# MisEty/RTG-SLAM

Hardware: AMD Instinct MI355X
Metric: hot_path_units_per_sec (higher is better)
Workload: dtype f32; 1 GPU; `value` counts UNITS, not SLAM frames (the SLAM frame rate by the reference's definition is `slam_frames_per_sec`, from the `slam_sequence` leg of --full).  One UNIT per step = 1 ICP track (3 levels x 5 GN iters, 1200x680, on a second HIP stream) + 1 map-optimisation iteration (raster fwd + masked L1 colour / gated depth loss + attach regulariser + raster bwd + fused Adam) over 1200000 random Gaus; gaussians=1200000, mode=single, parallelism=1 GPU

## Files before the change

### include/rtgs_icp.h

```cpp
#ifndef RTGS_ICP_H
#define RTGS_ICP_H

#include <stddef.h>
#include <stdint.h>

#ifdef __cplusplus
extern "C" {
#endif

#define RTGS_ICP_MAX_LEVELS 8


int rtgs_icp_build_pyramids(const float* depth, int32_t H, int32_t W, const float* K, int32_t levels,
                            float* const* vertex_out_host, float* const* normal_out_host,
                            void* scratch, void* stream);

int rtgs_icp_scratch_init(void* scratch, void* stream);
#define RTGS_ICP_PYR_SCRATCH_READY 1
#define RTGS_ICP_PYR_SECOND_SET 2
int rtgs_icp_build_pyramids_ex(const float* depth, int32_t H, int32_t W, const float* K, int32_t levels,
                               float* const* vertex_out_host, float* const* normal_out_host,
                               void* scratch, int32_t flags, void* stream);

int rtgs_icp_step(const float* vertex_src, const float* normal_src, const float* vertex_tgt,
                  const float* normal_tgt, int32_t H, int32_t W, const float* K, const float* pose,
                  float distance_threshold, float cos_normal_threshold,
                  float* JtJ_out, float* Jtr_out, float* nvalid_out, void* scratch, void* stream);

typedef struct rtgs_icp_level {
  int32_t H, W;
  float downscale;
  int32_t iters;
  const float* vertex_src;
  const float* normal_src;
  const float* vertex_tgt;
  const float* normal_tgt;
} rtgs_icp_level;

int rtgs_icp_track(const rtgs_icp_level* levels_host, int32_t n_levels, const float* K,
                   float distance_threshold, float cos_normal_threshold, float damping,
                   float* pose_inout, float* stats_out, void* scratch, int32_t flags, void* stream);
#define RTGS_ICP_FLAG_PERSISTENT 1
#define RTGS_ICP_FLAG_SCRATCH_READY 4
#define RTGS_ICP_FLAG_FROM_IDENTITY 8
#define RTGS_ICP_FLAG_F32_SOLVE 16
#define RTGS_ICP_FLAG_CLUSTER 2

int rtgs_icp_fill_model_depth(float* render_depth, const float* frame_depth, const float* render_normal,
                              const float* frame_normal, int32_t H, int32_t W, float dist_thr,
                              float normal_thr, void* stream);

size_t rtgs_icp_scratch_bytes(void);

#ifdef __cplusplus
}
#endif
#endif
```

### rtg_slam_amd/csrc/icp.hip

```cpp
#include "../../include/rtgs_icp.h"
#include "../../include/rtgs_debug.h"
#include <hip/hip_runtime.h>
#include <math.h>
#include <stdlib.h>

namespace rtgs_icp {

#ifndef RTGS_ICP_MAX_BLOCKS
#define RTGS_ICP_MAX_BLOCKS 256
#endif
constexpr int MAX_BLOCKS = RTGS_ICP_MAX_BLOCKS;
static_assert(MAX_BLOCKS <= RTGS_ICP_STAMP_WGS, "stamp slots hold RTGS_ICP_STAMP_WGS workgroups");
constexpr int NACC = 28;
constexpr int PSTRIDE = 32;

struct Scratch {
  uint32_t minmax[2 * RTGS_ICP_MAX_LEVELS];
  float partials[MAX_BLOCKS * PSTRIDE];
  uint32_t ticket;
  uint32_t pad[15];
  double sums[24 * 8 * PSTRIDE];
  unsigned long long dbg[96];
  uint32_t minmax_b[2 * RTGS_ICP_MAX_LEVELS];
};

#ifndef RTGS_ICP_WAVE_PRIO
#define RTGS_ICP_WAVE_PRIO 3
#endif
__device__ __forceinline__ void wave_priority_high() {
#if RTGS_ICP_WAVE_PRIO > 0
  __builtin_amdgcn_s_setprio(RTGS_ICP_WAVE_PRIO);
#endif
}

__device__ __forceinline__ uint32_t enc_f(float f) {
  const uint32_t u = __float_as_uint(f);
  return (u & 0x80000000u) ? ~u : (u | 0x80000000u);
}
__device__ __forceinline__ float dec_f(uint32_t e) {
  return __uint_as_float((e & 0x80000000u) ? (e & 0x7fffffffu) : ~e);
}

struct PyrDesc {
  int levels;
  int H, W;
  int Hl[RTGS_ICP_MAX_LEVELS], Wl[RTGS_ICP_MAX_LEVELS], shift[RTGS_ICP_MAX_LEVELS];
  int block_start[RTGS_ICP_MAX_LEVELS + 1];
  float* vertex[RTGS_ICP_MAX_LEVELS];
  float* normal[RTGS_ICP_MAX_LEVELS];
  uint32_t* mm;
  uint32_t* mm_rearm;
};

__global__ void __launch_bounds__(256) icp_vertex_kernel(PyrDesc d, const float* __restrict__ depth,
                                                         const float* __restrict__ K, Scratch* sc) {
  __shared__ uint32_t s_mm[2 * RTGS_ICP_MAX_LEVELS];
  if (threadIdx.x < 2 * RTGS_ICP_MAX_LEVELS) s_mm[threadIdx.x] = 0xffffffffu;
  __syncthreads();
  const int total = d.block_start[d.levels];
  for (int chunk = blockIdx.x; chunk < total; chunk += gridDim.x) {
    int l = 0;
    while (l + 1 < d.levels && chunk >= d.block_start[l + 1]) ++l;
    const int Hl = d.Hl[l], Wl = d.Wl[l], sh = d.shift[l];
    const int idx = (chunk - d.block_start[l]) * 256 + (int)threadIdx.x;
    float dmax = 0.f;
    const bool live = idx < Hl * Wl;
    if (live) {
      const int y = idx / Wl, x = idx % Wl;
      const int f = 1 << sh;
      dmax = -INFINITY;
      for (int a = 0; a < f; ++a)
        for (int b = 0; b < f; ++b) dmax = fmaxf(dmax, depth[(size_t)(y * f + a) * d.W + (x * f + b)]);
      const float ds = 1.f / (float)f;
      const float fx = K[0] * ds, fy = K[4] * ds, cx = K[2] * ds, cy = K[5] * ds;
      float* v = d.vertex[l] + (size_t)idx * 3;
      v[0] = (((float)x - cx) / fx) * dmax;
// ... 111 lines not shown
    if ((threadIdx.x & 63) == 0 && a != 0xffffffffu) { atomicMin(&s_mm[2 * l], a); atomicMin(&s_mm[2 * l + 1], bq); }
  }
  __syncthreads();
  if (threadIdx.x < 6 && s_mm[threadIdx.x] != 0xffffffffu) atomicMin(&d.mm[threadIdx.x], s_mm[threadIdx.x]);
  if (d.mm_rearm && blockIdx.x == 0 && threadIdx.x < 6) d.mm_rearm[threadIdx.x] = 0xffffffffu;
}

__global__ void __launch_bounds__(256) icp_normal_kernel(PyrDesc d, const Scratch* sc) {
  wave_priority_high();
  int l = 0;
  while (l + 1 < d.levels && (int)blockIdx.x >= d.block_start[l + 1]) ++l;
  const int Hl = d.Hl[l], Wl = d.Wl[l];
  const int idx = ((int)blockIdx.x - d.block_start[l]) * 256 + (int)threadIdx.x;
  if (idx >= Hl * Wl) return;
  const int y = idx / Wl, x = idx % Wl;
  const float* V = d.vertex[l];
  const int ym = max(y - 1, 0), yp = min(y + 1, Hl - 1), xm = max(x - 1, 0), xp = min(x + 1, Wl - 1);
  float gx[3], gy[3];
#pragma unroll
  for (int c = 0; c < 3; ++c) {
    const float a00 = V[((size_t)ym * Wl + xm) * 3 + c], a01 = V[((size_t)ym * Wl + x) * 3 + c], a02 = V[((size_t)ym * Wl + xp) * 3 + c];
    const float a10 = V[((size_t)y * Wl + xm) * 3 + c], a12 = V[((size_t)y * Wl + xp) * 3 + c];
    const float a20 = V[((size_t)yp * Wl + xm) * 3 + c], a21 = V[((size_t)yp * Wl + x) * 3 + c], a22 = V[((size_t)yp * Wl + xp) * 3 + c];
    gx[c] = -a00 + a02 - 2.f * a10 + 2.f * a12 - a20 + a22;
    gy[c] = -a00 - 2.f * a01 - a02 + a20 + 2.f * a21 + a22;
  }
  float nx = __fmaf_rn(gy[1], gx[2], -(gy[2] * gx[1]));
  float ny = __fmaf_rn(gy[2], gx[0], -(gy[0] * gx[2]));
  float nz = __fmaf_rn(gy[0], gx[1], -(gy[1] * gx[0]));
  const float mag = sqrtf(__fmaf_rn(nz, nz, __fmaf_rn(ny, ny, nx * nx))) + 1e-8f;
  nx /= mag; ny /= mag; nz /= mag;
  const float dep = V[(size_t)idx * 3 + 2];
  const float dmin = dec_f(d.mm[2 * l]), dmax = dec_f(~d.mm[2 * l + 1]);
  if (dep <= dmin || dep >= dmax) { nx = 0.f; ny = 0.f; nz = 0.f; }
  float* N = d.normal[l] + (size_t)idx * 3;
  N[0] = nx; N[1] = ny; N[2] = nz;
}

template <int CTRL, int ROW_MASK = 0xf>
__device__ __forceinline__ float dpp_add(float v) {
  const int moved = __builtin_amdgcn_update_dpp(0, __float_as_int(v), CTRL, ROW_MASK, 0xf, false);
  return v + __int_as_float(moved);
}
__device__ __forceinline__ float wave_sum63(float v) {
  v = dpp_add<0xB1>(v);
  v = dpp_add<0x4E>(v);
  v = dpp_add<0x141>(v);
  v = dpp_add<0x140>(v);
  v = dpp_add<0x142, 0xa>(v);
  v = dpp_add<0x143, 0xc>(v);
  return v;
}

template <int NCOL>
__device__ __forceinline__ void block_write_partials(float (&acc)[NCOL], float* __restrict__ partials) {
  __shared__ float s_part[4 * PSTRIDE];
  const int lane = threadIdx.x & 63, wave = threadIdx.x >> 6;
#pragma unroll
  for (int k = 0; k < NCOL; ++k) {
    const float r = wave_sum63(acc[k]);
    if (lane == 63) s_part[wave * PSTRIDE + k] = r;
  }
  __syncthreads();
  if (threadIdx.x < NCOL) {
    const int k = threadIdx.x;
    __hip_atomic_store(&partials[(size_t)blockIdx.x * PSTRIDE + k],
                       (s_part[k] + s_part[PSTRIDE + k]) + (s_part[2 * PSTRIDE + k] + s_part[3 * PSTRIDE + k]),
                       __ATOMIC_RELAXED, __HIP_MEMORY_SCOPE_AGENT);
  }
}

__device__ __forceinline__ void block_add_totals(float (&acc)[NACC], double* __restrict__ totals) {
  __shared__ float s_part2[4 * PSTRIDE];
  const int lane = threadIdx.x & 63, wave = threadIdx.x >> 6;
#pragma unroll
  for (int k = 0; k < NACC; ++k) {
    const float r = wave_sum63(acc[k]);
    if (lane == 63) s_part2[wave * PSTRIDE + k] = r;
  }
  __syncthreads();
  if (threadIdx.x < NACC) {
    const int k = threadIdx.x;
    const float v = (s_part2[k] + s_part2[PSTRIDE + k]) + (s_part2[2 * PSTRIDE + k] + s_part2[3 * PSTRIDE + k]);
    if (v != 0.f) unsafeAtomicAdd(&totals[k], (double)v);
  }
}

enum { MODE_SOLVE = 0, MODE_EQUATIONS = 1, MODE_P2P = 2 };

__device__ __forceinline__ float ld_sc1(const float* p) {
  return __hip_atomic_load(p, __ATOMIC_RELAXED, __HIP_MEMORY_SCOPE_AGENT);
}

struct FinalArgs {
  int mode;
  float damping, inv_pixels;
  float* pose;
  float* stats;
  float* JtJ_out;
  float* Jtr_out;
  float* nvalid_out;
  int first;
  int f32_solve;
};

__device__ __forceinline__ void sum_partials(const float* __restrict__ partials, int nblocks, double* s_sum, double* s_tot) {
  {
    const int q = threadIdx.x & 7, grp = threadIdx.x >> 3;
    double a0 = 0.0, a1 = 0.0, a2 = 0.0, a3 = 0.0;
    if (q < 7) {
      constexpr int MAXR = (MAX_BLOCKS + 31) / 32;
      float t[MAXR][4];
#pragma unroll
      for (int i = 0; i < MAXR; ++i) {
        const int r = grp + 32 * i;
        if (r < nblocks) {
          const float* row = partials + (size_t)r * PSTRIDE + 4 * q;
          t[i][0] = ld_sc1(row); t[i][1] = ld_sc1(row + 1); t[i][2] = ld_sc1(row + 2); t[i][3] = ld_sc1(row + 3);
        } else {
          t[i][0] = t[i][1] = t[i][2] = t[i][3] = 0.f;
        }
      }
#pragma unroll
      for (int i = 0; i < MAXR; ++i) { a0 += (double)t[i][0]; a1 += (double)t[i][1]; a2 += (double)t[i][2]; a3 += (double)t[i][3]; }
    }
    s_sum[grp * PSTRIDE + 4 * q] = a0; s_sum[grp * PSTRIDE + 4 * q + 1] = a1;
    s_sum[grp * PSTRIDE + 4 * q + 2] = a2; s_sum[grp * PSTRIDE + 4 * q + 3] = a3;
  }
  __syncthreads();
  if (threadIdx.x < NACC) {
    double t = 0.0;
#pragma unroll
    for (int g = 0; g < 32; ++g) t += s_sum[g * PSTRIDE + threadIdx.x];
    s_tot[threadIdx.x] = t;
  }
  __syncthreads();
}

__device__ __forceinline__ bool gn_update(const double (&S)[NACC], float damping, const float (&pin)[16], float* pose) {
  double Hm[6][6], bvec[6];
#pragma unroll
  for (int r = 0; r < 6; ++r)
#pragma unroll
    for (int c = r; c < 6; ++c) {
      const int idx = r * 6 - (r * (r - 1)) / 2 + (c - r);
      Hm[r][c] = S[idx]; Hm[c][r] = S[idx];
    }
#pragma unroll
  for (int r = 0; r < 6; ++r) bvec[r] = S[21 + r];
  double tr = 0.0;
#pragma unroll
  for (int r = 0; r < 6; ++r) tr += Hm[r][r];
#pragma unroll
  for (int r = 0; r < 6; ++r) Hm[r][r] += tr * (double)damping;
  double L[6][6], inv[6];
  bool spd = true;
#pragma unroll
  for (int r = 0; r < 6; ++r) {
#pragma unroll
    for (int c = 0; c <= r; ++c) {
      double s = Hm[r][c];
#pragma unroll
      for (int m = 0; m < c; ++m) s -= L[r][m] * L[c][m];
      if (r == c) {
        spd = spd && (s > 0.0);
        L[r][r] = sqrt(s > 0.0 ? s : 1.0);
        inv[r] = 1.0 / L[r][r];
      } else {
        L[r][c] = s * inv[c];
      }
    }
  }
  if (!spd) return false;
  double yv[6], xi[6];
#pragma unroll
  for (int r = 0; r < 6; ++r) {
    double s = -bvec[r];
// ... 164 lines not shown
        const int lo = r < c ? r : c, hi = r < c ? c : r;
        fa.JtJ_out[r * 6 + c] = (float)S[lo * 6 - (lo * (lo - 1)) / 2 + (hi - lo)];
      }
      fa.Jtr_out[r] = (float)S[21 + r];
    }
    fa.nvalid_out[0] = (float)S[27];
    return;
  }
  if (fa.first & 1) { fa.stats[1] = 0.f; fa.stats[2] = 0.f; fa.stats[3] = 0.f; }
  if (fa.first & 2) {
#pragma unroll
    for (int k = 0; k < 16; ++k) fa.pose[k] = (k % 5 == 0) ? 1.f : 0.f;
  }
  fa.stats[0] = (float)(S[27] * (double)fa.inv_pixels);
  if (!(fa.f32_solve ? gn_update_f32(S, fa.damping, pin, fa.pose) : gn_update(S, fa.damping, pin, fa.pose))) fa.stats[2] += 1.f;
}

template <bool STAMP>
__device__ __forceinline__ void final_stage(const float* __restrict__ partials, int nblocks, const FinalArgs& fa,
                                            unsigned long long (&cyc)[2]) {
  __shared__ double s_sum[32 * PSTRIDE];
  __shared__ double s_tot[PSTRIDE];
  unsigned long long t0 = 0;
  if constexpr (STAMP) t0 = __builtin_readcyclecounter();
  float pin[16];
#pragma unroll
  for (int k = 0; k < 16; ++k) pin[k] = (k % 5 == 0) ? 1.f : 0.f;
  if (threadIdx.x == 0 && fa.mode == MODE_SOLVE && !(fa.first & 2)) {
#pragma unroll
    for (int k = 0; k < 16; ++k) pin[k] = fa.pose[k];
  }
  sum_partials(partials, nblocks, s_sum, s_tot);
  if constexpr (STAMP) { const unsigned long long t = __builtin_readcyclecounter(); cyc[0] = t - t0; t0 = t; }
  if (threadIdx.x != 0) return;
  final_solve_from(s_tot, fa, pin);
  if constexpr (STAMP) {
    asm volatile("s_waitcnt vmcnt(0)" ::: "memory");
    cyc[1] = __builtin_readcyclecounter() - t0;
  }
}

__device__ __forceinline__ bool arrive_and_elect_last(uint32_t* ticket) {
  __shared__ uint32_t s_is_last;
  asm volatile("s_waitcnt vmcnt(0)" ::: "memory");
  __syncthreads();
  if (threadIdx.x == 0) {
    const uint32_t t = __hip_atomic_fetch_add(ticket, 1u, __ATOMIC_RELAXED, __HIP_MEMORY_SCOPE_AGENT);
    const uint32_t last = (t == gridDim.x - 1) ? 1u : 0u;
    if (last) __hip_atomic_store(ticket, 0u, __ATOMIC_RELAXED, __HIP_MEMORY_SCOPE_AGENT);
    s_is_last = last;
  }
  __syncthreads();
  return s_is_last != 0;
}

struct LevelGeom {
  float R00, R01, R02, t0, R10, R11, R12, t1, R20, R21, R22, t2;
  float fx, fy, cx, cy, Wm1, Hm1, hw, hh, dist_thr, cos_thr;
  int W;
};

struct Proj {
  float px, py, pz;
  int j;
};
struct Tgt {
  float q0, q1, q2, m0, m1, m2;
};

__device__ __forceinline__ Proj project(const LevelGeom& g, float v0, float v1, float v2) {
  Proj P;
  P.px = (g.R00 * v0 + g.R01 * v1 + g.R02 * v2) + g.t0;
  P.py = (g.R10 * v0 + g.R11 * v1 + g.R12 * v2) + g.t1;
  P.pz = (g.R20 * v0 + g.R21 * v1 + g.R22 * v2) + g.t2;
  P.j = -1;
  const float u = (P.px / P.pz) * g.fx + g.cx;
  const float v = (P.py / P.pz) * g.fy + g.cy;
  const bool inview = (u > 0.f) && (u < g.Wm1) && (v > 0.f) && (v < g.Hm1);
  if (inview && (v2 > 0.f)) {
    const float un = u / g.hw - 1.f, vn = v / g.hh - 1.f;
    float ix = ((un + 1.f) / 2.f) * g.Wm1, iy = ((vn + 1.f) / 2.f) * g.Hm1;
    ix = fminf(g.Wm1, fmaxf(ix, 0.f));
    iy = fminf(g.Hm1, fmaxf(iy, 0.f));
    P.j = ((int)nearbyintf(iy) * g.W + (int)nearbyintf(ix)) * 3;
  }
  return P;
}

__device__ __forceinline__ Tgt gather(const Proj& P, const float* __restrict__ vt, const float* __restrict__ nt) {
  const int j = P.j < 0 ? 0 : P.j;
  return Tgt{vt[j], vt[j + 1], vt[j + 2], nt[j], nt[j + 1], nt[j + 2]};
}

__device__ __forceinline__ void finish(const LevelGeom& g, const Proj& P, float n0, float n1, float n2, const Tgt& T,
                                       float (&acc)[NACC]) {
  if (P.j < 0 || !(T.q2 > 0.f)) return;
  const float rn0 = g.R00 * n0 + g.R01 * n1 + g.R02 * n2;
  const float rn1 = g.R10 * n0 + g.R11 * n1 + g.R12 * n2;
  const float rn2 = g.R20 * n0 + g.R21 * n1 + g.R22 * n2;
  if (!(rn0 * T.m0 + rn1 * T.m1 + rn2 * T.m2 > g.cos_thr)) return;
  const float d0 = P.px - T.q0, d1 = P.py - T.q1, d2 = P.pz - T.q2;
  if (sqrtf(d0 * d0 + d1 * d1 + d2 * d2) > g.dist_thr) return;
  const float r = T.m0 * d0 + T.m1 * d1 + T.m2 * d2;
  float J[6];
  J[0] = P.py * T.m2 - P.pz * T.m1;
  J[1] = P.pz * T.m0 - P.px * T.m2;
// ... 66 lines not shown
  if (idx < n) {
    const float* v = vs + (size_t)idx * 3;
    const float* m = ns + (size_t)idx * 3;
    const float n0 = m[0], n1 = m[1], n2 = m[2];
    const Proj P = project(g, v[0], v[1], v[2]);
    finish(g, P, n0, n1, n2, gather(P, vt, nt), acc);
  }
}

template <bool STAMP>
__device__ __forceinline__ void icp_reduce_body(
    const float* __restrict__ vs, const float* __restrict__ ns, const float* __restrict__ vt,
    const float* __restrict__ nt, int H, int W, const float* __restrict__ K, float ds,
    const float* __restrict__ pose, float dist_thr, float cos_thr, float* __restrict__ partials,
    uint32_t* __restrict__ ticket, const FinalArgs& fa, unsigned long long* __restrict__ stamps) {
  wave_priority_high();
  unsigned long long wall0 = 0;
  Stamp st{0, 0, 0, 0};
  if constexpr (STAMP) { wall0 = wall_clock64(); st.t = __builtin_readcyclecounter(); }
  const LevelGeom g = make_geom((fa.first & 2) ? c_identity : pose, K, ds, H, W, dist_thr, cos_thr);
  float acc[NACC];
#pragma unroll
  for (int k = 0; k < NACC; ++k) acc[k] = 0.f;
  accumulate_range<STAMP>(g, vs, ns, vt, nt, H * W, blockIdx.x * 256 + threadIdx.x, gridDim.x * 256, acc, st);
  block_write_partials<NACC>(acc, partials);
  const bool last = arrive_and_elect_last(ticket);
  unsigned long long pub = 0, fin[2] = {0, 0};
  stamp_lap<STAMP>(st, pub, false);
  if (last) final_stage<STAMP>(partials, (int)gridDim.x, fa, fin);
  if constexpr (STAMP) {
    if ((threadIdx.x & 63) == 0) {
      unsigned long long* o = stamps + ((size_t)blockIdx.x * 4 + (threadIdx.x >> 6)) * 8;
      o[0] = wall0; o[1] = wall_clock64(); o[2] = st.src; o[3] = st.gat; o[4] = st.acc; o[5] = pub;
      o[6] = fin[0]; o[7] = fin[1];
    }
  }
}

#define RTGS_ICP_REDUCE_ARGS                                                                                              \
  const float *__restrict__ vs, const float *__restrict__ ns, const float *__restrict__ vt,                               \
      const float *__restrict__ nt, int H, int W, const float *__restrict__ K, float ds, const float *__restrict__ pose,  \
      float dist_thr, float cos_thr, float *__restrict__ partials, uint32_t *__restrict__ ticket, FinalArgs fa,          \
      unsigned long long *__restrict__ stamps
#define RTGS_ICP_REDUCE_PASS vs, ns, vt, nt, H, W, K, ds, pose, dist_thr, cos_thr, partials, ticket, fa, stamps
__global__ void __launch_bounds__(256) icp_reduce_kernel(RTGS_ICP_REDUCE_ARGS) {
  icp_reduce_body<false>(RTGS_ICP_REDUCE_PASS);
}
__global__ void __launch_bounds__(256) icp_reduce_stamped_kernel(RTGS_ICP_REDUCE_ARGS) {
  icp_reduce_body<true>(RTGS_ICP_REDUCE_PASS);
}
#undef RTGS_ICP_REDUCE_ARGS
#undef RTGS_ICP_REDUCE_PASS

constexpr int P2P_QUADS = 2;
__device__ __forceinline__ float p2p_term(const float* Rt, float v0, float v1, float v2, float q0, float q1, float q2,
                                          float m0, float m1, float m2) {
  const float px = (v0 * Rt[0] + v1 * Rt[1] + v2 * Rt[2]) + Rt[3];
  const float py = (v0 * Rt[4] + v1 * Rt[5] + v2 * Rt[6]) + Rt[7];
  const float pz = (v0 * Rt[8] + v1 * Rt[9] + v2 * Rt[10]) + Rt[11];
  const float l = (px - q0) * m0 + (py - q1) * m1 + (pz - q2) * m2;
  return l * l;
}

__global__ void __launch_bounds__(256) icp_p2p_kernel(const float* __restrict__ vs, const float* __restrict__ vt,
                                                      const float* __restrict__ nt, int n,
                                                      const float* __restrict__ pose, float* __restrict__ partials,
                                                      uint32_t* __restrict__ ticket, FinalArgs fa) {
  wave_priority_high();
  float Rt[12];
#pragma unroll
  for (int k = 0; k < 12; ++k) Rt[k] = pose[k];
  float acc[1] = {0.f};
  const int n4 = n >> 2, first = blockIdx.x * 256 + threadIdx.x, stride = gridDim.x * 256;
  const float4* vs4 = reinterpret_cast<const float4*>(vs);
  const float4* vt4 = reinterpret_cast<const float4*>(vt);
  const float4* nt4 = reinterpret_cast<const float4*>(nt);
  for (int base = first; base < n4; base += P2P_QUADS * stride) {
    float4 a[P2P_QUADS][3], c[P2P_QUADS][3], m[P2P_QUADS][3];
#pragma unroll
    for (int i = 0; i < P2P_QUADS; ++i) {
      const int q = base + i * stride;
      if (q < n4) {
#pragma unroll
        for (int k = 0; k < 3; ++k) { a[i][k] = vs4[3 * q + k]; c[i][k] = vt4[3 * q + k]; m[i][k] = nt4[3 * q + k]; }
      }
    }
#pragma unroll
    for (int i = 0; i < P2P_QUADS; ++i) {
      if (base + i * stride >= n4) break;
      acc[0] += p2p_term(Rt, a[i][0].x, a[i][0].y, a[i][0].z, c[i][0].x, c[i][0].y, c[i][0].z, m[i][0].x, m[i][0].y, m[i][0].z);
      acc[0] += p2p_term(Rt, a[i][0].w, a[i][1].x, a[i][1].y, c[i][0].w, c[i][1].x, c[i][1].y, m[i][0].w, m[i][1].x, m[i][1].y);
      acc[0] += p2p_term(Rt, a[i][1].z, a[i][1].w, a[i][2].x, c[i][1].z, c[i][1].w, c[i][2].x, m[i][1].z, m[i][1].w, m[i][2].x);
      acc[0] += p2p_term(Rt, a[i][2].y, a[i][2].z, a[i][2].w, c[i][2].y, c[i][2].z, c[i][2].w, m[i][2].y, m[i][2].z, m[i][2].w);
    }
  }
  const int idx = 4 * n4 + first;
  if (idx < n) {
    const size_t j = (size_t)idx * 3;
    acc[0] += p2p_term(Rt, vs[j], vs[j + 1], vs[j + 2], vt[j], vt[j + 1], vt[j + 2], nt[j], nt[j + 1], nt[j + 2]);
  }
  block_write_partials<1>(acc, partials);
  unsigned long long fin[2];
  if (arrive_and_elect_last(ticket)) final_stage<false>(partials, (int)gridDim.x, fa, fin);
}
struct TrackLevel {
  const float *vs, *ns, *vt, *nt;
  int H, W, iters;
  float ds;
};
struct TrackArgs {
  TrackLevel lv[RTGS_ICP_MAX_LEVELS];
  int n_levels;
  const float* K;
  float dist_thr, cos_thr, damping;
  float* pose;
  float* stats;
  double* sums;
  uint32_t* ticket;
  uint32_t* abort_flag;
  unsigned long long* dbg;
  int cluster, levels_here;
};

__device__ __forceinline__ bool grid_arrive_wait(uint32_t* ticket, uint32_t target, uint32_t* abort_flag, float* stats) {
  __shared__ int s_ok;
  asm volatile("s_waitcnt vmcnt(0)" ::: "memory");
  __syncthreads();
  if (threadIdx.x == 0) {
    __hip_atomic_fetch_add(ticket, 1u, __ATOMIC_RELAXED, __HIP_MEMORY_SCOPE_AGENT);
    int ok = 0;
    for (int spin = 0; spin < (1 << 22); ++spin) {
      if (__hip_atomic_load(ticket, __ATOMIC_RELAXED, __HIP_MEMORY_SCOPE_AGENT) >= target) { ok = 1; break; }
      if ((spin & 63) == 63 && __hip_atomic_load(abort_flag, __ATOMIC_RELAXED, __HIP_MEMORY_SCOPE_AGENT) != 0u) break;
      __builtin_amdgcn_s_sleep(1);
    }
    if (!ok) {
      __hip_atomic_store(abort_flag, 1u, __ATOMIC_RELAXED, __HIP_MEMORY_SCOPE_AGENT);
      stats[3] = 1.f;
    }
    s_ok = ok;
  }
  __syncthreads();
  return s_ok != 0;
}

__device__ __forceinline__ double load_totals(const double* totals, int k) {
  double t[8];
#pragma unroll
  for (int r = 0; r < 8; ++r) t[r] = __hip_atomic_load(&totals[r * PSTRIDE + k], __ATOMIC_RELAXED, __HIP_MEMORY_SCOPE_AGENT);
  return ((t[0] + t[1]) + (t[2] + t[3])) + ((t[4] + t[5]) + (t[6] + t[7]));
}

__global__ void __launch_bounds__(256) icp_track_kernel(TrackArgs a) {
// ... 68 lines not shown
      const float py = (v0 * R10 + v1 * R11 + v2 * R12) + t1;
      const float pz = (v0 * R20 + v1 * R21 + v2 * R22) + t2;
      const float lp = (px - F.vt[j]) * F.nt[j] + (py - F.vt[j + 1]) * F.nt[j + 1] + (pz - F.vt[j + 2]) * F.nt[j + 2];
      acc[0] += lp * lp;
    }
    double* totals = a.sums + (size_t)epoch * 8 * PSTRIDE;
    block_add_totals(acc, totals + ((uint32_t)bid & 7u) * PSTRIDE);
    ++epoch;
    if (!grid_arrive_wait(a.ticket, epoch * (uint32_t)G, a.abort_flag, a.stats)) return;
    if (bid != 0) return;
    if (threadIdx.x < 12) a.pose[threadIdx.x] = s_pose[threadIdx.x];
    if (threadIdx.x == 0) {
      a.stats[0] = s_stat[0];
      a.stats[1] = (float)(load_totals(totals, 0) * (1.0 / (double)n));
      a.stats[2] = s_stat[2];
    }
  }
}

__global__ void __launch_bounds__(256) icp_fill_kernel(float* __restrict__ rd, const float* __restrict__ fd,
                                                       const float* __restrict__ rn, const float* __restrict__ fn,
                                                       int n, float dist_thr, float normal_thr) {
  const int i = blockIdx.x * 256 + threadIdx.x;
  if (i >= n) return;
  const float r = rd[i], f = fd[i];
  const float a0 = rn[3 * i], a1 = rn[3 * i + 1], a2 = rn[3 * i + 2];
  const float b0 = fn[3 * i], b1 = fn[3 * i + 1], b2 = fn[3 * i + 2];
  const float na = fmaxf(sqrtf(a0 * a0 + a1 * a1 + a2 * a2), 1e-8f);
  const float nb = fmaxf(sqrtf(b0 * b0 + b1 * b1 + b2 * b2), 1e-8f);
  const float cs = (a0 / na) * (b0 / nb) + (a1 / na) * (b1 / nb) + (a2 / na) * (b2 / nb);
  const bool fill = ((fabsf(r - f) > dist_thr) || (r == 0.f) || ((1.f - cs) > normal_thr)) && (f > 0.f);
  if (fill) rd[i] = f;
}

static int grid_for(int n) {
  int g = (n + 255) / 256;
  return g > MAX_BLOCKS ? MAX_BLOCKS : (g < 1 ? 1 : g);
}

static unsigned long long* g_stamps = nullptr;
static int g_stamp_launch = 0;

static void launch_reduce(const float* vs, const float* ns, const float* vt, const float* nt, int H, int W, const float* K,
                          float ds, const float* pose, float dist_thr, float cos_thr, float* partials, uint32_t* ticket,
                          const FinalArgs& fa, hipStream_t st) {
  const int g = grid_for((H * W + 3) / 4);
  unsigned long long* stamps = nullptr;
  if (g_stamps) stamps = g_stamps + (size_t)(g_stamp_launch++ % RTGS_ICP_STAMP_LAUNCHES) * RTGS_ICP_STAMP_WGS * 4 * 8;
#define RTGS_ICP_LAUNCH(KERNEL)                                                                                        \
  hipLaunchKernelGGL(KERNEL, dim3(g), dim3(256), 0, st, vs, ns, vt, nt, H, W, K, ds, pose, dist_thr, cos_thr, partials, \
                     ticket, fa, stamps)
  if (stamps) RTGS_ICP_LAUNCH(icp_reduce_stamped_kernel); else RTGS_ICP_LAUNCH(icp_reduce_kernel);
#undef RTGS_ICP_LAUNCH
}

}

using namespace rtgs_icp;

#define ICP_TRY(expr)                \
  do {                               \
    if ((expr) != hipSuccess) return -2; \
  } while (0)

extern "C" {

size_t rtgs_icp_scratch_bytes(void) { return sizeof(Scratch); }

int rtgs_icp_build_pyramids(const float* depth, int32_t H, int32_t W, const float* K, int32_t levels,
                            float* const* vertex_out, float* const* normal_out, void* scratch, void* stream) {
  return rtgs_icp_build_pyramids_ex(depth, H, W, K, levels, vertex_out, normal_out, scratch, 0, stream);
}

int rtgs_icp_scratch_init(void* scratch, void* stream) {
  if (!scratch) return -1;
  Scratch* sc = (Scratch*)scratch;
  hipStream_t st = (hipStream_t)stream;
  ICP_TRY(hipMemsetAsync(sc, 0, sizeof(Scratch), st));
  ICP_TRY(hipMemsetAsync(sc->minmax, 0xff, sizeof(sc->minmax), st));
  ICP_TRY(hipMemsetAsync(sc->minmax_b, 0xff, sizeof(sc->minmax_b), st));
  return 0;
}

int rtgs_icp_build_pyramids_ex(const float* depth, int32_t H, int32_t W, const float* K, int32_t levels,
                               float* const* vertex_out, float* const* normal_out, void* scratch, int32_t flags,
                               void* stream) {
  if (!depth || !K || !vertex_out || !normal_out || !scratch || H <= 0 || W <= 0 || levels < 1 ||
      levels > RTGS_ICP_MAX_LEVELS)
    return -1;
  hipStream_t st = (hipStream_t)stream;
  Scratch* sc = (Scratch*)scratch;
  PyrDesc d{};
  d.levels = levels; d.H = H; d.W = W;
  int blocks = 0;
  for (int l = 0; l < levels; ++l) {
    const int sh = levels - 1 - l;
    d.shift[l] = sh; d.Hl[l] = H >> sh; d.Wl[l] = W >> sh;
    if (d.Hl[l] < 1 || d.Wl[l] < 1 || !vertex_out[l] || !normal_out[l]) return -1;
    d.vertex[l] = vertex_out[l]; d.normal[l] = normal_out[l];
    d.block_start[l] = blocks;
    blocks += (d.Hl[l] * d.Wl[l] + 255) / 256;
  }
  d.block_start[levels] = blocks;
  if (flags & RTGS_ICP_PYR_SCRATCH_READY) {
    const bool second = (flags & RTGS_ICP_PYR_SECOND_SET) != 0;
    d.mm = second ? sc->minmax_b : sc->minmax;
// ... 47 lines not shown
  const int cluster = env_cluster >= 0 ? env_cluster : ((flags & RTGS_ICP_FLAG_CLUSTER) ? 64 : 0);
  if ((flags & RTGS_ICP_FLAG_F32_SOLVE) && (persistent || (cluster > 0 && n_levels >= 2))) return -1;
  const bool plain = !persistent && !(cluster > 0 && n_levels >= 2);
  if (!(plain && ready)) {
    ICP_TRY(hipMemsetAsync(stats, 0, 4 * sizeof(float), st));
    ICP_TRY(hipMemsetAsync(&sc->ticket, 0, 2 * sizeof(uint32_t), st));
  }
  if (from_identity && !plain) {
    static const float eye[16] = {1.f, 0.f, 0.f, 0.f, 0.f, 1.f, 0.f, 0.f, 0.f, 0.f, 1.f, 0.f, 0.f, 0.f, 0.f, 1.f};
    ICP_TRY(hipMemcpyAsync(pose, eye, sizeof(eye), hipMemcpyHostToDevice, st));
  }
  if (persistent) {
    int dev = 0, cus = 0;
    ICP_TRY(hipGetDevice(&dev));
    ICP_TRY(hipDeviceGetAttribute(&cus, hipDeviceAttributeMultiprocessorCount, dev));
    int G = cus > 0 ? cus : 64;
    if (G > MAX_BLOCKS) G = MAX_BLOCKS;
    TrackArgs a{};
    for (int l = 0; l < n_levels; ++l)
      a.lv[l] = TrackLevel{lv[l].vertex_src, lv[l].normal_src, lv[l].vertex_tgt, lv[l].normal_tgt, lv[l].H, lv[l].W,
                           lv[l].iters, lv[l].downscale};
    a.n_levels = n_levels; a.K = K; a.dist_thr = dist_thr; a.cos_thr = cos_thr; a.damping = damping;
    a.pose = pose; a.stats = stats; a.sums = sc->sums; a.ticket = &sc->ticket; a.abort_flag = &sc->pad[0];
    int n_barriers = 1;
    for (int l = 0; l < n_levels; ++l) n_barriers += lv[l].iters;
    if (n_barriers > 24) return -1;
    ICP_TRY(hipMemsetAsync(sc->sums, 0, (size_t)n_barriers * 8 * PSTRIDE * sizeof(double), st));
    static const bool dbg_timing = [] { const char* e = getenv("RTGS_ICP_DEBUG_TIMING"); return e && atoi(e) != 0; }();
    a.dbg = dbg_timing ? sc->dbg : nullptr;
    hipLaunchKernelGGL(icp_track_kernel, dim3(G), dim3(256), 0, st, a);
    ICP_TRY(hipMemsetAsync(&sc->ticket, 0, 2 * sizeof(uint32_t), st));
    ICP_TRY(hipGetLastError());
    return 0;
  }
  int first_launched = 0;
  if (cluster > 0 && n_levels >= 2) {
    TrackArgs a{};
    int n_barriers = 0;
    for (int l = 0; l < n_levels - 1; ++l) {
      a.lv[l] = TrackLevel{lv[l].vertex_src, lv[l].normal_src, lv[l].vertex_tgt, lv[l].normal_tgt, lv[l].H, lv[l].W,
                           lv[l].iters, lv[l].downscale};
      n_barriers += lv[l].iters;
    }
    if (n_barriers > 24) return -1;
    a.n_levels = n_levels; a.K = K; a.dist_thr = dist_thr; a.cos_thr = cos_thr; a.damping = damping;
    a.pose = pose; a.stats = stats; a.sums = sc->sums; a.ticket = &sc->ticket; a.abort_flag = &sc->pad[0];
    a.dbg = nullptr;
    a.cluster = cluster > 64 ? 64 : cluster; a.levels_here = n_levels - 1;
    ICP_TRY(hipMemsetAsync(sc->sums, 0, (size_t)(n_barriers + 1) * 8 * PSTRIDE * sizeof(double), st));
    hipLaunchKernelGGL(icp_track_kernel, dim3(8 * a.cluster), dim3(256), 0, st, a);
    ICP_TRY(hipMemsetAsync(&sc->ticket, 0, sizeof(uint32_t), st));
    first_launched = n_levels - 1;
  }
  bool launched_any = false;
  for (int l = first_launched; l < n_levels; ++l) {
    const rtgs_icp_level& L = lv[l];
    const float inv = 1.f / ((float)L.H * (float)L.W);
    FinalArgs fa{(int)MODE_SOLVE, damping, inv, pose, stats, nullptr, nullptr, nullptr, 0, (flags & RTGS_ICP_FLAG_F32_SOLVE) ? 1 : 0};
    for (int it = 0; it < L.iters; ++it) {
      fa.first = (plain && !launched_any) ? (1 | (from_identity ? 2 : 0)) : 0;
      launched_any = true;
      launch_reduce(L.vertex_src, L.normal_src, L.vertex_tgt, L.normal_tgt, L.H, L.W, K, L.downscale, pose, dist_thr,
                    cos_thr, sc->partials, &sc->ticket, fa, st);
    }
  }
  if (plain && !launched_any) {
    ICP_TRY(hipMemsetAsync(stats, 0, 4 * sizeof(float), st));
    if (from_identity) {
      static const float eye0[16] = {1.f, 0.f, 0.f, 0.f, 0.f, 1.f, 0.f, 0.f, 0.f, 0.f, 1.f, 0.f, 0.f, 0.f, 0.f, 1.f};
      ICP_TRY(hipMemcpyAsync(pose, eye0, sizeof(eye0), hipMemcpyHostToDevice, st));
    }
  }
  const rtgs_icp_level& F = lv[n_levels - 1];
  const int n = F.H * F.W;
  const int g = grid_for((n + 3) / 4);
  FinalArgs fp{(int)MODE_P2P, 0.f, 1.f / (float)n, pose, stats, nullptr, nullptr, nullptr, 0, 0};
  hipLaunchKernelGGL(icp_p2p_kernel, dim3(g), dim3(256), 0, st, F.vertex_src, F.vertex_tgt, F.normal_tgt, n,
                     (const float*)pose, sc->partials, &sc->ticket, fp);
  ICP_TRY(hipGetLastError());
  return 0;
}

void rtgs_icp_set_stamps(void* dev) {
  g_stamps = (unsigned long long*)dev;
  g_stamp_launch = 0;
}

int rtgs_icp_fill_model_depth(float* rd, const float* fd, const float* rn, const float* fn, int32_t H, int32_t W,
                              float dist_thr, float normal_thr, void* stream) {
  if (!rd || !fd || !rn || !fn || H <= 0 || W <= 0) return -1;
  const int n = H * W;
  hipLaunchKernelGGL(icp_fill_kernel, dim3((n + 255) / 256), dim3(256), 0, (hipStream_t)stream, rd, fd, rn, fn, n,
                     dist_thr, normal_thr);
  ICP_TRY(hipGetLastError());
  return 0;
}

}
```

### rtg_slam_amd/icp.py

```python
from __future__ import annotations

import ctypes as C
from typing import List, Sequence, Tuple

import numpy as np
import torch

from . import _lib


def _require_device(t: torch.Tensor):
    if not t.is_cuda:
        raise RuntimeError("rtg_slam_amd.icp: tensors must live on a HIP device; this build has no CPU path.")


def _f32c(t: torch.Tensor) -> torch.Tensor:
    if t.dtype != torch.float32:
        t = t.float()
    return t.contiguous()


def _vp(t: torch.Tensor):
    return C.c_void_p(t.data_ptr())


_scratch = {}
_builds = {}
FLAG_PERSISTENT, FLAG_CLUSTER, FLAG_SCRATCH_READY, FLAG_FROM_IDENTITY, FLAG_F32_SOLVE = 1, 2, 4, 8, 16
PYR_SCRATCH_READY, PYR_SECOND_SET = 1, 2


def _scratch_key(dev):
    return (dev.type, dev.index, torch.cuda.current_stream(dev).cuda_stream)


def _get_scratch(dev) -> torch.Tensor:
    key = _scratch_key(dev)
    s = _scratch.get(key)
    if s is None:
        lib = _lib.load()
        s = torch.empty(lib.rtgs_icp_scratch_bytes(), dtype=torch.uint8, device=dev)
        with torch.cuda.device(dev):
            _lib.check(lib.rtgs_icp_scratch_init(_vp(s), C.c_void_p(key[2])), "rtgs_icp_scratch_init")
        _scratch[key] = s
        _builds[key] = 0
    return s


def build_pyramids(depth: torch.Tensor, K: torch.Tensor, levels: int = 3) -> Tuple[List[torch.Tensor], List[torch.Tensor]]:
    lib = _lib.load()
    _require_device(depth)
    dev = depth.device
    depth = _f32c(depth)
    H, W = int(depth.shape[0]), int(depth.shape[1])
    K = _f32c(K.to(dev))
    verts, norms = [], []
    for l in range(levels):
        sh = levels - 1 - l
        verts.append(torch.empty(H >> sh, W >> sh, 3, dtype=torch.float32, device=dev))
        norms.append(torch.empty(H >> sh, W >> sh, 3, dtype=torch.float32, device=dev))
    vp = (C.c_void_p * levels)(*[v.data_ptr() for v in verts])
    npp = (C.c_void_p * levels)(*[n.data_ptr() for n in norms])
    stream = torch.cuda.current_stream(dev).cuda_stream
    scratch = _get_scratch(dev)
    key = _scratch_key(dev)
    flags = PYR_SCRATCH_READY | (PYR_SECOND_SET if _builds[key] & 1 else 0)
    with torch.cuda.device(dev):
        rc = lib.rtgs_icp_build_pyramids_ex(_vp(depth), H, W, _vp(K), levels, vp, npp, _vp(scratch), flags,
                                            C.c_void_p(stream))
    _lib.check(rc, "rtgs_icp_build_pyramids_ex")
    _builds[key] += 1
    return verts, norms


def icp_step(v_src, n_src, v_tgt, n_tgt, K, pose, dist_thr: float, cos_thr: float):
    lib = _lib.load()
    _require_device(v_src)
    dev = v_src.device
    v_src, n_src, v_tgt, n_tgt = map(_f32c, (v_src, n_src, v_tgt, n_tgt))
    H, W = int(v_src.shape[0]), int(v_src.shape[1])
    K = _f32c(K.to(dev))
    pose = _f32c(pose.to(dev))
    JtJ = torch.empty(6, 6, dtype=torch.float32, device=dev)
    Jtr = torch.empty(6, dtype=torch.float32, device=dev)
    nv = torch.empty(1, dtype=torch.float32, device=dev)
    stream = torch.cuda.current_stream(dev).cuda_stream
    with torch.cuda.device(dev):
        rc = lib.rtgs_icp_step(_vp(v_src), _vp(n_src), _vp(v_tgt), _vp(n_tgt), H, W, _vp(K), _vp(pose),
                               float(dist_thr), float(cos_thr), _vp(JtJ), _vp(Jtr), _vp(nv),
                               _vp(_get_scratch(dev)), C.c_void_p(stream))
    _lib.check(rc, "rtgs_icp_step")
    return JtJ, Jtr, nv


def icp_track(vertex_src: Sequence[torch.Tensor], normal_src, vertex_tgt, normal_tgt, K: torch.Tensor,
              downscales: Sequence[float], iters: Sequence[int], dist_thr: float, cos_thr: float,
              damping: float, pose0: torch.Tensor | None = None, persistent: bool = False,
              f32_solve: bool = False) -> torch.Tensor:
    lib = _lib.load()
    dev = vertex_src[0].device
    _require_device(vertex_src[0])
    n = len(downscales)
    keep = []
    lv = (_lib.IcpLevelC * n)()
    for l in range(n):
        ts = [_f32c(t[l]) for t in (vertex_src, normal_src, vertex_tgt, normal_tgt)]
        keep.append(ts)
        lv[l] = _lib.IcpLevelC(int(ts[0].shape[0]), int(ts[0].shape[1]), float(downscales[l]), int(iters[l]),
                               ts[0].data_ptr(), ts[1].data_ptr(), ts[2].data_ptr(), ts[3].data_ptr())
    K = _f32c(K.to(dev))
    out = torch.empty(20, dtype=torch.float32, device=dev)
    flags = (FLAG_PERSISTENT if persistent else 0) | FLAG_SCRATCH_READY | (FLAG_F32_SOLVE if f32_solve else 0)
    if pose0 is None:
        flags |= FLAG_FROM_IDENTITY
    else:
        out[:16] = _f32c(pose0.to(dev)).reshape(-1)
    stream = torch.cuda.current_stream(dev).cuda_stream
    with torch.cuda.device(dev):
        rc = lib.rtgs_icp_track(lv, n, _vp(K), float(dist_thr), float(cos_thr), float(damping),
                                C.c_void_p(out.data_ptr()), C.c_void_p(out.data_ptr() + 64),
                                _vp(_get_scratch(dev)), flags, C.c_void_p(stream))
    _lib.check(rc, "rtgs_icp_track")
    return out


def fill_model_depth(render_depth, frame_depth, render_normal, frame_normal, dist_thr: float, normal_thr: float):
    lib = _lib.load()
    _require_device(render_depth)
    if render_depth.dtype != torch.float32 or not render_depth.is_contiguous():
        raise RuntimeError("render_depth must be a contiguous float32 tensor (it is updated in place)")
    dev = render_depth.device
    H, W = int(render_depth.shape[0]), int(render_depth.shape[1])
    fd, rn, fn = _f32c(frame_depth), _f32c(render_normal), _f32c(frame_normal)
    stream = torch.cuda.current_stream(dev).cuda_stream
    with torch.cuda.device(dev):
        rc = lib.rtgs_icp_fill_model_depth(_vp(render_depth), _vp(fd), _vp(rn), _vp(fn), H, W, float(dist_thr),
                                           float(normal_thr), C.c_void_p(stream))
    _lib.check(rc, "rtgs_icp_fill_model_depth")
    return render_depth


class IcpTracker:

    def __init__(self, args):
        self.icp_downscales = list(args.icp_downscales)
        self.icp_warmup_frames = args.icp_warmup_frames
        self.icp_use_model_depth = args.icp_use_model_depth
        self.icp_downscale_iters = list(args.icp_downscale_iters)
        self.icp_distance_threshold = float(args.icp_distance_threshold)
        self.icp_normal_threshold = float(np.cos(np.deg2rad(args.icp_normal_threshold)))
        self.icp_damping = float(args.icp_damping)
        self.icp_sample_distance_threshold = args.icp_sample_distance_threshold
        self.icp_sample_normal_threshold = args.icp_sample_normal_threshold
        self.icp_fail_threshold = args.icp_fail_threshold
        self.verbose = getattr(args, "verbose", False)
        self.persistent = bool(getattr(args, "icp_persistent", False))
        n = len(self.icp_downscales)
        for l, ds in enumerate(self.icp_downscales):
            if abs(ds - 1.0 / (1 << (n - 1 - l))) > 1e-12:
                raise ValueError("icp_downscales must be [2^-(n-1), ..., 0.5, 1.0] (SLAM/icp.py:374)")
        self.normal_pyramid_t0 = None
        self.vertex_pyramid_t0 = None
        self.normal_pyramid_t1 = None
        self.vertex_pyramid_t1 = None
        self.last_model_depth = None
# ... 58 lines not shown
```

Baseline: 2873 units/s.

## Replace last-arriver reduction with redundant per-block head solve in next kernel

In the plain ICP tracking path, each Gauss-Newton iteration's kernel now starts by summing the previous launch's per-block partials and redundantly solving the 6x6 update in every workgroup. This removes the atomic ticket and last-block election. Partials are double-buffered across launches, so plain stores and float4 loads replace the agent-scope atomic stores and loads. The cost is extra redundant head work per block (partials reduction plus solve) and a serialized prologue before accumulation. The old last-arriver path stays reachable through a flag or environment variable.

Result: faster. 2905 units/s (median of 6 runs) (+1.1%).

```diff
diff --git a/include/rtgs_icp.h b/include/rtgs_icp.h
--- a/include/rtgs_icp.h
+++ b/include/rtgs_icp.h
@@ -44,6 +44,7 @@
 #define RTGS_ICP_FLAG_SCRATCH_READY 4
 #define RTGS_ICP_FLAG_FROM_IDENTITY 8
 #define RTGS_ICP_FLAG_F32_SOLVE 16
+#define RTGS_ICP_FLAG_LAST_ARRIVER 32
 #define RTGS_ICP_FLAG_CLUSTER 2
 
 int rtgs_icp_fill_model_depth(float* render_depth, const float* frame_depth, const float* render_normal,
diff --git a/rtg_slam_amd/csrc/icp.hip b/rtg_slam_amd/csrc/icp.hip
--- a/rtg_slam_amd/csrc/icp.hip
+++ b/rtg_slam_amd/csrc/icp.hip
@@ -22,6 +22,8 @@
   double sums[24 * 8 * PSTRIDE];
   unsigned long long dbg[96];
   uint32_t minmax_b[2 * RTGS_ICP_MAX_LEVELS];
+  float partials_b[MAX_BLOCKS * PSTRIDE];
+  float pose_slots[2][16];
 };
 
 #ifndef RTGS_ICP_WAVE_PRIO
@@ -239,7 +241,7 @@
   return v;
 }
 
-template <int NCOL>
+template <int NCOL, bool SC1 = true>
 __device__ __forceinline__ void block_write_partials(float (&acc)[NCOL], float* __restrict__ partials) {
   __shared__ float s_part[4 * PSTRIDE];
   const int lane = threadIdx.x & 63, wave = threadIdx.x >> 6;
@@ -251,9 +253,9 @@
   __syncthreads();
   if (threadIdx.x < NCOL) {
     const int k = threadIdx.x;
-    __hip_atomic_store(&partials[(size_t)blockIdx.x * PSTRIDE + k],
-                       (s_part[k] + s_part[PSTRIDE + k]) + (s_part[2 * PSTRIDE + k] + s_part[3 * PSTRIDE + k]),
-                       __ATOMIC_RELAXED, __HIP_MEMORY_SCOPE_AGENT);
+    const float v = (s_part[k] + s_part[PSTRIDE + k]) + (s_part[2 * PSTRIDE + k] + s_part[3 * PSTRIDE + k]);
+    if constexpr (SC1) __hip_atomic_store(&partials[(size_t)blockIdx.x * PSTRIDE + k], v, __ATOMIC_RELAXED, __HIP_MEMORY_SCOPE_AGENT);
+    else partials[(size_t)blockIdx.x * PSTRIDE + k] = v;
   }
 }
 
@@ -291,6 +293,7 @@
   int f32_solve;
 };
 
+template <bool SC1 = true>
 __device__ __forceinline__ void sum_partials(const float* __restrict__ partials, int nblocks, double* s_sum, double* s_tot) {
   {
     const int q = threadIdx.x & 7, grp = threadIdx.x >> 3;
@@ -303,13 +306,21 @@
         const int r = grp + 32 * i;
         if (r < nblocks) {
           const float* row = partials + (size_t)r * PSTRIDE + 4 * q;
-          t[i][0] = ld_sc1(row); t[i][1] = ld_sc1(row + 1); t[i][2] = ld_sc1(row + 2); t[i][3] = ld_sc1(row + 3);
+          if constexpr (SC1) {
+            t[i][0] = ld_sc1(row); t[i][1] = ld_sc1(row + 1); t[i][2] = ld_sc1(row + 2); t[i][3] = ld_sc1(row + 3);
+          } else {
+            const float4 v = *reinterpret_cast<const float4*>(row);
+            t[i][0] = v.x; t[i][1] = v.y; t[i][2] = v.z; t[i][3] = v.w;
+          }
         } else {
           t[i][0] = t[i][1] = t[i][2] = t[i][3] = 0.f;
         }
       }
 #pragma unroll
-      for (int i = 0; i < MAXR; ++i) { a0 += (double)t[i][0]; a1 += (double)t[i][1]; a2 += (double)t[i][2]; a3 += (double)t[i][3]; }
+      for (int i = 0; i < MAXR; ++i) {
+        if (!SC1 && 32 * i >= nblocks) break;
+        a0 += (double)t[i][0]; a1 += (double)t[i][1]; a2 += (double)t[i][2]; a3 += (double)t[i][3];
+      }
     }
     s_sum[grp * PSTRIDE + 4 * q] = a0; s_sum[grp * PSTRIDE + 4 * q + 1] = a1;
     s_sum[grp * PSTRIDE + 4 * q + 2] = a2; s_sum[grp * PSTRIDE + 4 * q + 3] = a3;
@@ -580,6 +591,61 @@
   }
   __syncthreads();
   return s_is_last != 0;
+}
+
+struct HeadArgs {
+  const float* partials;
+  int rows;
+  float inv_pixels;
+  float damping;
+  const float* pose_in;
+  float* pose_out;
+  float* stats;
+  int first;
+  int f32_solve;
+};
+
+template <bool STAMP>
+__device__ __forceinline__ void head_consume(const HeadArgs& h, float* s_pose, unsigned long long (&cyc)[2]) {
+  __shared__ double s_hsum[32 * PSTRIDE];
+  __shared__ double s_htot[PSTRIDE];
+  if (h.partials == nullptr) {
+    if (threadIdx.x < 16) {
+      const float v = (h.first & 2) ? ((threadIdx.x % 5 == 0) ? 1.f : 0.f) : h.pose_in[threadIdx.x];
+      s_pose[threadIdx.x] = v;
+      if (blockIdx.x == 0) h.pose_out[threadIdx.x] = v;
+    }
+    if (blockIdx.x == 0 && threadIdx.x == 0) { h.stats[1] = 0.f; h.stats[2] = 0.f; h.stats[3] = 0.f; }
+    __syncthreads();
+    return;
+  }
+  unsigned long long t0 = 0;
+  if constexpr (STAMP) t0 = __builtin_readcyclecounter();
+  float pin[16];
+#pragma unroll
+  for (int k = 0; k < 16; ++k) pin[k] = 0.f;
+  if (threadIdx.x == 0) {
+#pragma unroll
+    for (int k = 0; k < 16; ++k) pin[k] = h.pose_in[k];
+  }
+  sum_partials<false>(h.partials, h.rows, s_hsum, s_htot);
+  if constexpr (STAMP) { const unsigned long long t = __builtin_readcyclecounter(); cyc[0] = t - t0; t0 = t; }
+  if (threadIdx.x == 0) {
+    double S[NACC];
+#pragma unroll
+    for (int c = 0; c < NACC; ++c) S[c] = s_htot[c];
+#pragma unroll
+    for (int k = 0; k < 16; ++k) s_pose[k] = pin[k];
+    const bool ok = h.f32_solve ? gn_update_f32(S, h.damping, pin, s_pose) : gn_update(S, h.damping, pin, s_pose);
+    if (blockIdx.x == 0) {
+#pragma unroll
+      for (int k = 0; k < 16; ++k) h.pose_out[k] = s_pose[k];
+      h.stats[0] = (float)(S[27] * (double)h.inv_pixels);
+      if (!ok) h.stats[2] += 1.f;
+    }
+  }
+  __syncthreads();
+  if constexpr (STAMP) cyc[1] = __builtin_readcyclecounter() - t0;
 }
 
 struct LevelGeom {
@@ -752,6 +818,49 @@
 #undef RTGS_ICP_REDUCE_ARGS
 #undef RTGS_ICP_REDUCE_PASS
 
+template <bool STAMP>
+__device__ __forceinline__ void icp_reduce_head_body(
+    const float* __restrict__ vs, const float* __restrict__ ns, const float* __restrict__ vt,
+    const float* __restrict__ nt, int H, int W, const float* __restrict__ K, float ds, float dist_thr, float cos_thr,
+    float* __restrict__ partials, const HeadArgs& h, unsigned long long* __restrict__ stamps) {
+  wave_priority_high();
+  __shared__ float s_pose[16];
+  unsigned long long wall0 = 0;
+  Stamp st{0, 0, 0, 0};
+  if constexpr (STAMP) wall0 = wall_clock64();
+  unsigned long long head[2] = {0, 0};
+  head_consume<STAMP>(h, s_pose, head);
+  if constexpr (STAMP) st.t = __builtin_readcyclecounter();
+  const LevelGeom g = make_geom(s_pose, K, ds, H, W, dist_thr, cos_thr);
+  float acc[NACC];
+#pragma unroll
+  for (int k = 0; k < NACC; ++k) acc[k] = 0.f;
+  accumulate_range<STAMP>(g, vs, ns, vt, nt, H * W, blockIdx.x * 256 + threadIdx.x, gridDim.x * 256, acc, st);
+  block_write_partials<NACC, false>(acc, partials);
+  unsigned long long pub = 0;
+  stamp_lap<STAMP>(st, pub, true);
+  if constexpr (STAMP) {
+    if ((threadIdx.x & 63) == 0) {
+      unsigned long long* o = stamps + ((size_t)blockIdx.x * 4 + (threadIdx.x >> 6)) * 8;
+      o[0] = wall0; o[1] = wall_clock64(); o[2] = st.src; o[3] = st.gat; o[4] = st.acc; o[5] = pub;
+      o[6] = head[0]; o[7] = head[1];
+    }
+  }
+}
+#define RTGS_ICP_REDUCE_ARGS                                                                                            \
+  const float *__restrict__ vs, const float *__restrict__ ns, const float *__restrict__ vt,                             \
+      const float *__restrict__ nt, int H, int W, const float *__restrict__ K, float ds, float dist_thr, float cos_thr, \
+      float *__restrict__ partials, HeadArgs h, unsigned long long *__restrict__ stamps
+#define RTGS_ICP_REDUCE_PASS vs, ns, vt, nt, H, W, K, ds, dist_thr, cos_thr, partials, h, stamps
+__global__ void __launch_bounds__(256) icp_reduce_head_kernel(RTGS_ICP_REDUCE_ARGS) {
+  icp_reduce_head_body<false>(RTGS_ICP_REDUCE_PASS);
+}
+__global__ void __launch_bounds__(256) icp_reduce_head_stamped_kernel(RTGS_ICP_REDUCE_ARGS) {
+  icp_reduce_head_body<true>(RTGS_ICP_REDUCE_PASS);
+}
+#undef RTGS_ICP_REDUCE_ARGS
+#undef RTGS_ICP_REDUCE_PASS
+
 constexpr int P2P_QUADS = 2;
 __device__ __forceinline__ float p2p_term(const float* Rt, float v0, float v1, float v2, float q0, float q1, float q2,
                                           float m0, float m1, float m2) {
@@ -762,6 +871,38 @@
   return l * l;
 }
 
+__device__ __forceinline__ void p2p_accumulate(const float (&Rt)[12], const float* __restrict__ vs, const float* __restrict__ vt,
+                                               const float* __restrict__ nt, int n, float (&acc)[1]) {
+  const int n4 = n >> 2, first = blockIdx.x * 256 + threadIdx.x, stride = gridDim.x * 256;
+  const float4* vs4 = reinterpret_cast<const float4*>(vs);
+  const float4* vt4 = reinterpret_cast<const float4*>(vt);
+  const float4* nt4 = reinterpret_cast<const float4*>(nt);
+  for (int base = first; base < n4; base += P2P_QUADS * stride) {
+    float4 a[P2P_QUADS][3], c[P2P_QUADS][3], m[P2P_QUADS][3];
+#pragma unroll
+    for (int i = 0; i < P2P_QUADS; ++i) {
+      const int q = base + i * stride;
+      if (q < n4) {
+#pragma unroll
+        for (int k = 0; k < 3; ++k) { a[i][k] = vs4[3 * q + k]; c[i][k] = vt4[3 * q + k]; m[i][k] = nt4[3 * q + k]; }
+      }
+    }
+#pragma unroll
+    for (int i = 0; i < P2P_QUADS; ++i) {
+      if (base + i * stride >= n4) break;
+      acc[0] += p2p_term(Rt, a[i][0].x, a[i][0].y, a[i][0].z, c[i][0].x, c[i][0].y, c[i][0].z, m[i][0].x, m[i][0].y, m[i][0].z);
+      acc[0] += p2p_term(Rt, a[i][0].w, a[i][1].x, a[i][1].y, c[i][0].w, c[i][1].x, c[i][1].y, m[i][0].w, m[i][1].x, m[i][1].y);
+      acc[0] += p2p_term(Rt, a[i][1].z, a[i][1].w, a[i][2].x, c[i][1].z, c[i][1].w, c[i][2].x, m[i][1].z, m[i][1].w, m[i][2].x);
+      acc[0] += p2p_term(Rt, a[i][2].y, a[i][2].z, a[i][2].w, c[i][2].y, c[i][2].z, c[i][2].w, m[i][2].y, m[i][2].z, m[i][2].w);
+    }
+  }
+  const int idx = 4 * n4 + first;
+  if (idx < n) {
+    const size_t j = (size_t)idx * 3;
+    acc[0] += p2p_term(Rt, vs[j], vs[j + 1], vs[j + 2], vt[j], vt[j + 1], vt[j + 2], nt[j], nt[j + 1], nt[j + 2]);
+  }
+}
+
 __global__ void __launch_bounds__(256) icp_p2p_kernel(const float* __restrict__ vs, const float* __restrict__ vt,
                                                       const float* __restrict__ nt, int n,
                                                       const float* __restrict__ pose, float* __restrict__ partials,
@@ -771,34 +912,25 @@
 #pragma unroll
   for (int k = 0; k < 12; ++k) Rt[k] = pose[k];
   float acc[1] = {0.f};
-  const int n4 = n >> 2, first = blockIdx.x * 256 + threadIdx.x, stride = gridDim.x * 256;
-  const float4* vs4 = reinterpret_cast<const float4*>(vs);
-  const float4* vt4 = reinterpret_cast<const float4*>(vt);
-  const float4* nt4 = reinterpret_cast<const float4*>(nt);
-  for (int base = first; base < n4; base += P2P_QUADS * stride) {
-    float4 a[P2P_QUADS][3], c[P2P_QUADS][3], m[P2P_QUADS][3];
-#pragma unroll
-    for (int i = 0; i < P2P_QUADS; ++i) {
-      const int q = base + i * stride;
-      if (q < n4) {
-#pragma unroll
-        for (int k = 0; k < 3; ++k) { a[i][k] = vs4[3 * q + k]; c[i][k] = vt4[3 * q + k]; m[i][k] = nt4[3 * q + k]; }
-      }
-    }
-#pragma unroll
-    for (int i = 0; i < P2P_QUADS; ++i) {
-      if (base + i * stride >= n4) break;
-      acc[0] += p2p_term(Rt, a[i][0].x, a[i][0].y, a[i][0].z, c[i][0].x, c[i][0].y, c[i][0].z, m[i][0].x, m[i][0].y, m[i][0].z);
-      acc[0] += p2p_term(Rt, a[i][0].w, a[i][1].x, a[i][1].y, c[i][0].w, c[i][1].x, c[i][1].y, m[i][0].w, m[i][1].x, m[i][1].y);
-      acc[0] += p2p_term(Rt, a[i][1].z, a[i][1].w, a[i][2].x, c[i][1].z, c[i][1].w, c[i][2].x, m[i][1].z, m[i][1].w, m[i][2].x);
-      acc[0] += p2p_term(Rt, a[i][2].y, a[i][2].z, a[i][2].w, c[i][2].y, c[i][2].z, c[i][2].w, m[i][2].y, m[i][2].z, m[i][2].w);
-    }
-  }
-  const int idx = 4 * n4 + first;
-  if (idx < n) {
-    const size_t j = (size_t)idx * 3;
-    acc[0] += p2p_term(Rt, vs[j], vs[j + 1], vs[j + 2], vt[j], vt[j + 1], vt[j + 2], nt[j], nt[j + 1], nt[j + 2]);
-  }
+  p2p_accumulate(Rt, vs, vt, nt, n, acc);
+  block_write_partials<1>(acc, partials);
+  unsigned long long fin[2];
+  if (arrive_and_elect_last(ticket)) final_stage<false>(partials, (int)gridDim.x, fa, fin);
+}
+
+__global__ void __launch_bounds__(256) icp_p2p_head_kernel(const float* __restrict__ vs, const float* __restrict__ vt,
+                                                           const float* __restrict__ nt, int n,
+                                                           float* __restrict__ partials, uint32_t* __restrict__ ticket,
+                                                           FinalArgs fa, HeadArgs h) {
+  wave_priority_high();
+  __shared__ float s_pose[16];
+  unsigned long long cyc[2];
+  head_consume<false>(h, s_pose, cyc);
+  float Rt[12];
+#pragma unroll
+  for (int k = 0; k < 12; ++k) Rt[k] = s_pose[k];
+  float acc[1] = {0.f};
+  p2p_accumulate(Rt, vs, vt, nt, n, acc);
   block_write_partials<1>(acc, partials);
   unsigned long long fin[2];
   if (arrive_and_elect_last(ticket)) final_stage<false>(partials, (int)gridDim.x, fa, fin);
@@ -973,6 +1105,20 @@
                      ticket, fa, stamps)
   if (stamps) RTGS_ICP_LAUNCH(icp_reduce_stamped_kernel); else RTGS_ICP_LAUNCH(icp_reduce_kernel);
 #undef RTGS_ICP_LAUNCH
+}
+
+static int launch_reduce_head(const float* vs, const float* ns, const float* vt, const float* nt, int H, int W,
+                              const float* K, float ds, float dist_thr, float cos_thr, float* partials,
+                              const HeadArgs& h, hipStream_t st) {
+  const int g = grid_for((H * W + 3) / 4);
+  unsigned long long* stamps = nullptr;
+  if (g_stamps) stamps = g_stamps + (size_t)(g_stamp_launch++ % RTGS_ICP_STAMP_LAUNCHES) * RTGS_ICP_STAMP_WGS * 4 * 8;
+#define RTGS_ICP_LAUNCH(KERNEL)                                                                                     \
+  hipLaunchKernelGGL(KERNEL, dim3(g), dim3(256), 0, st, vs, ns, vt, nt, H, W, K, ds, dist_thr, cos_thr, partials, h, \
+                     stamps)
+  if (stamps) RTGS_ICP_LAUNCH(icp_reduce_head_stamped_kernel); else RTGS_ICP_LAUNCH(icp_reduce_head_kernel);
+#undef RTGS_ICP_LAUNCH
+  return g;
 }
 
 }
@@ -1126,6 +1272,47 @@
     ICP_TRY(hipMemsetAsync(&sc->ticket, 0, sizeof(uint32_t), st));
     first_launched = n_levels - 1;
   }
+  static const int env_last_arriver = [] { const char* e = getenv("RTGS_ICP_LAST_ARRIVER"); return e ? (atoi(e) != 0 ? 1 : 0) : -1; }();
+  const bool last_arriver = env_last_arriver >= 0 ? env_last_arriver == 1 : (flags & RTGS_ICP_FLAG_LAST_ARRIVER) != 0;
+  if (plain && !last_arriver) {
+    float* bufs[2] = {sc->partials, sc->partials_b};
+    HeadArgs h{nullptr, 0, 0.f, damping, pose, nullptr, stats, 1 | (from_identity ? 2 : 0), (flags & RTGS_ICP_FLAG_F32_SOLVE) ? 1 : 0};
+    int j = 0;
+    for (int l = 0; l < n_levels; ++l) {
+      const rtgs_icp_level& L = lv[l];
+      for (int it = 0; it < L.iters; ++it) {
+        ++j;
+        h.pose_out = sc->pose_slots[(j + 1) & 1];
+        h.rows = launch_reduce_head(L.vertex_src, L.normal_src, L.vertex_tgt, L.normal_tgt, L.H, L.W, K, L.downscale,
+                                    dist_thr, cos_thr, bufs[j & 1], h, st);
+        h.partials = bufs[j & 1];
+        h.inv_pixels = 1.f / ((float)L.H * (float)L.W);
+        h.pose_in = h.pose_out;
+        h.first = 0;
+      }
+    }
+    const rtgs_icp_level& F = lv[n_levels - 1];
+    const int n = F.H * F.W;
+    const int g = grid_for((n + 3) / 4);
+    if (j == 0) {
+      ICP_TRY(hipMemsetAsync(stats, 0, 4 * sizeof(float), st));
+      if (from_identity) {
+        static const float eye1[16] = {1.f, 0.f, 0.f, 0.f, 0.f, 1.f, 0.f, 0.f, 0.f, 0.f, 1.f, 0.f, 0.f, 0.f, 0.f, 1.f};
+        ICP_TRY(hipMemcpyAsync(pose, eye1, sizeof(eye1), hipMemcpyHostToDevice, st));
+      }
+      FinalArgs fp{(int)MODE_P2P, 0.f, 1.f / (float)n, pose, stats, nullptr, nullptr, nullptr, 0, 0};
+      hipLaunchKernelGGL(icp_p2p_kernel, dim3(g), dim3(256), 0, st, F.vertex_src, F.vertex_tgt, F.normal_tgt, n,
+                         (const float*)pose, sc->partials, &sc->ticket, fp);
+    } else {
+      ++j;
+      h.pose_out = pose;
+      FinalArgs fp{(int)MODE_P2P, 0.f, 1.f / (float)n, nullptr, stats, nullptr, nullptr, nullptr, 0, 0};
+      hipLaunchKernelGGL(icp_p2p_head_kernel, dim3(g), dim3(256), 0, st, F.vertex_src, F.vertex_tgt, F.normal_tgt, n,
+                         bufs[j & 1], &sc->ticket, fp, h);
+    }
+    ICP_TRY(hipGetLastError());
+    return 0;
+  }
   bool launched_any = false;
   for (int l = first_launched; l < n_levels; ++l) {
     const rtgs_icp_level& L = lv[l];
diff --git a/rtg_slam_amd/icp.py b/rtg_slam_amd/icp.py
--- a/rtg_slam_amd/icp.py
+++ b/rtg_slam_amd/icp.py
@@ -26,7 +26,7 @@
 
 _scratch = {}
 _builds = {}
-FLAG_PERSISTENT, FLAG_CLUSTER, FLAG_SCRATCH_READY, FLAG_FROM_IDENTITY, FLAG_F32_SOLVE = 1, 2, 4, 8, 16
+FLAG_PERSISTENT, FLAG_CLUSTER, FLAG_SCRATCH_READY, FLAG_FROM_IDENTITY, FLAG_F32_SOLVE, FLAG_LAST_ARRIVER = 1, 2, 4, 8, 16, 32
 PYR_SCRATCH_READY, PYR_SECOND_SET = 1, 2
 
 
@@ -96,7 +96,7 @@
 def icp_track(vertex_src: Sequence[torch.Tensor], normal_src, vertex_tgt, normal_tgt, K: torch.Tensor,
               downscales: Sequence[float], iters: Sequence[int], dist_thr: float, cos_thr: float,
               damping: float, pose0: torch.Tensor | None = None, persistent: bool = False,
-              f32_solve: bool = False) -> torch.Tensor:
+              f32_solve: bool = False, last_arriver: bool = False) -> torch.Tensor:
     lib = _lib.load()
     dev = vertex_src[0].device
     _require_device(vertex_src[0])
@@ -111,6 +111,7 @@
     K = _f32c(K.to(dev))
     out = torch.empty(20, dtype=torch.float32, device=dev)
     flags = (FLAG_PERSISTENT if persistent else 0) | FLAG_SCRATCH_READY | (FLAG_F32_SOLVE if f32_solve else 0)
+    flags |= FLAG_LAST_ARRIVER if last_arriver else 0
     if pose0 is None:
         flags |= FLAG_FROM_IDENTITY
     else:
```
